# kentsommer/2D-EKF-SLAM

Measured on AMD Instinct MI355X. Metric: EKF steps/sec (propagate+full update) at N landmarks, higher is better.
Workload: dtype f64

## Files before the change

### 2d-ekf-slam_amd/csrc/ekf_api.hip

```cpp
#include <math.h>
#include <stdio.h>
#include <stdlib.h>
#include <string.h>
#include <time.h>

#include <string>
#include <atomic>
#include <mutex>
#include <functional>
#include <vector>
#include <algorithm>

#include "ekf_device.h"
#include "ekf_geometry.h"

#include "ekf_kernels.hip"
#include "ekf_solo.hip"
#include "ekf_rewrite.hip"
#include "ekf_factor.hip"
#include "ekf_pairs.hip"

static thread_local std::string g_last_error;

static int set_error(int code, const char *what) {
// ... 139 lines not shown

extern "C" void ekf_default_params(ekf_params *p) {
    if (!p) return;
    p->sigma_v = 0.01;
    p->sigma_w = 0.04;
    p->gamma_max = 50.0;
    p->gamma_min = 10.0;
    p->cond_limit = 80.0;
    p->max_pending = 16;
    p->log_capacity = 4096;
    p->overlap = -1;
}

static EnvInt env_int(const char *name) {
    EnvInt e;
    if (const char *s = getenv(name)) e.set = true, e.v = atoi(s);
    return e;
}

struct ProcessTunables {
    bool trace;
    bool inline_rec;
};
static const ProcessTunables &process_tunables() {
    static const ProcessTunables t = {env_int("EKF_TRACE").v != 0, env_int("EKF_INLINE_REC").flag(true)};
    return t;
}
static bool trace_on() { return process_tunables().trace; }

static Tunables read_tunables() {
    Tunables t;
    t.overlap = env_int("EKF_OVERLAP");
    t.solo = env_int("EKF_SOLO");
    t.chain_wgs = env_int("EKF_CHAIN_WGS");
    t.solo_long_window = env_int("EKF_SOLO_LONG_WINDOW");
    t.solo_fuse = env_int("EKF_SOLO_FUSE");
    t.chain_one = env_int("EKF_CHAIN_ONE");
    t.chain_helpers = env_int("EKF_CHAIN_HELPERS");
    t.solo_stagger_ticks = env_int("EKF_SOLO_STAGGER_US").set ? env_int("EKF_SOLO_STAGGER_US").v * 100 : 3500;
    t.bm_skew_bytes = getenv("EKF_BM_SKEW") ? atol(getenv("EKF_BM_SKEW")) : 4096;
    t.stream_ring_host = env_int("EKF_STREAM_RING_HOST").flag(false);
    t.balanced_tail = env_int("EKF_BALANCED_TAIL").flag(true);
    t.chain_cus = env_int("EKF_CHAIN_CUS");
    t.inkernel_wait = env_int("EKF_INKERNEL_WAIT").flag(true);
    t.solo_groups = env_int("EKF_SOLO_GROUPS").or_else(1);
    t.flush_alternate = env_int("EKF_FLUSH_ALTERNATE").flag(true);
    t.persist = env_int("EKF_PERSIST").flag(true);
    t.stream = env_int("EKF_STREAM").flag(true);
    t.xcd_map = env_int("EKF_XCD_MAP").flag(true);
    t.batch_interleave = env_int("EKF_BATCH_INTERLEAVE").flag(true);
    t.overlap_serial = getenv("EKF_OVERLAP_SERIAL") != nullptr;
    t.solo_fuse_stagger_ticks = env_int("EKF_SOLO_FUSE_STAGGER_US").v * 100;
    t.inline_rec = process_tunables().inline_rec;
    return t;
}
#define TRACE(msg)                                          \
    do {                                                    \
        if (trace_on()) {                                   \
            fprintf(stderr, "[ekf] %s\n", msg);             \
            fflush(stderr);                                 \
        }                                                   \
    } while (0)

struct PooledStream {
    int device, keep;
    hipStream_t s;
};
static std::mutex g_pool_mu;
static std::vector<PooledStream> g_pool;

static bool pool_take(int device, int keep, hipStream_t *out) {
    std::lock_guard<std::mutex> lk(g_pool_mu);
    for (size_t i = 0; i < g_pool.size(); i++)
        if (g_pool[i].device == device && g_pool[i].keep == keep) {
            *out = g_pool[i].s;
            g_pool.erase(g_pool.begin() + i);
            return true;
        }
    return false;
}

static void pool_drain() {
    std::lock_guard<std::mutex> lk(g_pool_mu);
    for (auto &p : g_pool) {
        if (hipSetDevice(p.device) == hipSuccess) hipStreamDestroy(p.s);
    }
    g_pool.clear();
}

static void pool_give(int device, int keep, hipStream_t s) {
    static bool registered = false;
    std::lock_guard<std::mutex> lk(g_pool_mu);
    if (!registered) {
        atexit(pool_drain);
        registered = true;
    }
    g_pool.push_back({device, keep, s});
}

static int concurrent_kernels_ok(int device, hipStream_t a, hipStream_t b) {
    static std::mutex mu;
    static std::vector<int> cache(64, -1);
    std::lock_guard<std::mutex> lk(mu);
    if (device >= 0 && device < (int)cache.size() && cache[device] >= 0) return cache[device];
    int h[2] = {0, 0}, ok = 0;
    {
// ... 136 lines not shown
    int ndev = 0;
    if (hipGetDeviceCount(&ndev) != hipSuccess || ndev <= 0)
        return set_error(EKF_ERR_NO_DEVICE, "no HIP device: libekfslam_hip has no CPU fallback");
    if (device_id < 0 || device_id >= ndev || device_id >= 64) return set_error(EKF_ERR_BAD_ARG, "bad device_id");
    hipDeviceProp_t prop;
    HIP_TRY(hipGetDeviceProperties(&prop, device_id));
    if (strncmp(prop.gcnArchName, "gfx950", 6) != 0) {
        char buf[256];
        snprintf(buf, sizeof buf, "device %d is %s; this library carries gfx950 code objects only", device_id, prop.gcnArchName);
        return set_error(EKF_ERR_NO_DEVICE, buf);
    }
    HIP_TRY(hipSetDevice(device_id));
    ekf_batch *h = new ekf_batch();
    h->device = device_id;
    int rc = create_impl(h, batch, capacity_landmarks, device_id, params, prop);
    if (rc != EKF_OK) {
        std::string keep = g_last_error;
        ekf_destroy(h);
        (void)hipGetLastError();
        g_last_error = keep;
        return rc;
    }
    *out = h;
    return EKF_OK;
}

static int create_impl(ekf_batch *h, int batch, int capacity_landmarks, int device_id, const ekf_params *params, const hipDeviceProp_t &prop) {
    ekf_default_params(&h->params);
    if (params) h->params = *params;
    h->params_requested = h->params;
    if (h->params.log_capacity < 16) h->params.log_capacity = 16;

    h->tn = read_tunables();
    const Tunables &tn = h->tn;
    const ChainGeometry geo = plan_geometry(batch, capacity_landmarks, h->params, prop.sharedMemPerBlock, tn);
    if (geo.error) return set_error(geo.error, geo.what);
    h->params.max_pending = geo.max_pending;
    h->params.overlap = geo.overlap ? 1 : 0;
    h->overlap = geo.overlap;
    h->solo = geo.solo, h->solo_kernel = geo.solo_kernel, h->solo_long = geo.solo_long, h->solo_fuse = geo.solo_fuse;
    h->chain_wgs = geo.chain_wgs, h->chain_filters = geo.chain_filters, h->chain_threads = geo.chain_threads;
    h->chain_lds = geo.chain_lds, h->chain_one = geo.chain_one;
    EkfDev &dv = h->dv;
    memset(&dv, 0, sizeof dv);
    dv.B = batch;
    dv.Ncap = capacity_landmarks;
    dv.T = geo.T, dv.xs = geo.xs, dv.dn = geo.dn, dv.rows = geo.rows, dv.bm_stride = geo.bm_stride;
    dv.maxp = geo.max_pending, dv.maxpairs = geo.maxpairs, dv.f_stride = geo.f_stride, dv.vs_cap = geo.cache_slots;
    dv.gmax = geo.chain_wgs, dv.lpw = geo.lpw, dv.hpw = geo.hpw, dv.nrec = geo.nrec;
    dv.logcap = h->params.log_capacity;
    dv.gamma_max = h->params.gamma_max;
    dv.gamma_min = h->params.gamma_min;
    dv.spin_limit = 1LL << 24;
    dv.cond_limit = h->params.cond_limit;
    {
        const long double L = h->params.cond_limit;
        long double kappa = L <= 1.0L ? 0.0L : 0.5L - 1.0L / (L * L + 1.0L);
        dv.cond_k2 = (double)(kappa * kappa);
    }

    for (int k = 0; k < 8; k++)
        HIP_TRY(hipFuncSetAttribute((const void *)chain_kernel((k & 4) != 0, (k & 2) != 0, (k & 1) != 0), hipFuncAttributeMaxDynamicSharedMemorySize,
                                    (int)chain_lds_budget(prop.sharedMemPerBlock)));
    {
        const int G = h->chain_wgs;
        int per_cu = 0;
        HIP_TRY(hipOccupancyMaxActiveBlocksPerMultiprocessor(&per_cu, (const void *)chain_kernel(h, false), h->chain_threads, h->chain_lds));
        if (per_cu < 1) return set_error(EKF_ERR_STATE, "the chain kernel does not fit a CU with this capacity / window");
        const int need = h->solo ? 0 : (G * h->chain_filters + per_cu - 1) / per_cu;
        std::lock_guard<std::mutex> lk(g_res_mu);
        if (g_cus_claimed[device_id] + need > prop.multiProcessorCount) {
            char buf[256];
            snprintf(buf, sizeof buf, "this handle's %d chain workgroups need %d CUs, %d of %d are claimed by live handles: they could not all be resident at once",
                     G * h->chain_filters, need, g_cus_claimed[device_id], prop.multiProcessorCount);
            return set_error(EKF_ERR_STATE, buf);
        }
        g_cus_claimed[device_id] += need;
        h->claimed_cus = need;
        h->solo_cus = h->solo ? (h->chain_filters + per_cu - 1) / per_cu : 0;
        if (h->solo_cus > prop.multiProcessorCount) h->solo_cus = prop.multiProcessorCount;
        g_cus_solo[device_id] += h->solo_cus;
        h->ncu = prop.multiProcessorCount;
    }

    if (!pool_take(device_id, -1, &h->s_chain)) {
        TRACE("create: stream");
        HIP_TRY(hipStreamCreateWithFlags(&h->s_chain, hipStreamNonBlocking));
        TRACE("create: stream done");
    }
    const size_t B = batch;
    hipStream_t s = h->s_chain;
    for (const DevArray &a : device_arrays(h)) {
        HIP_TRY(dev_alloc_zero_bytes(a.slot, a.count(batch), a.elem, &h->device_bytes, s));
        if (a.slot != (void **)&dv.Bm[0]) continue;
        if (h->overlap) {
            const size_t skew = (size_t)tn.bm_skew_bytes / sizeof(double);
            HIP_TRY(dev_alloc_zero(&h->bm1_base, B * dv.bm_stride + skew, &h->device_bytes, s));
            dv.Bm[1] = h->bm1_base + skew;
        }
        else dv.Bm[1] = dv.Bm[0];
    }
    TRACE("create: device buffers queued");
    HIP_TRY(hipHostMalloc((void **)&h->mirror_h, B * sizeof(EkfMirror), hipHostMallocMapped));
    memset(h->mirror_h, 0, B * sizeof(EkfMirror));
    HIP_TRY(hipHostGetDevicePointer((void **)&dv.mirror, h->mirror_h, 0));
    HIP_TRY(hipHostMalloc((void **)&h->sctl_h, sizeof(StreamCtl), hipHostMallocMapped));
// ... 1839 lines not shown
```

### 2d-ekf-slam_amd/csrc/ekf_device.h

```cpp
#pragma once
#include <hip/hip_runtime.h>
#include <hip/hip_ext.h>
#include <stdint.h>

#include "../../include/ekfslam_c.h"

#define EKF_INF 999999999999.0
#define EKF_MAX_PENDING 32
#define EKF_MAX_PAIRS (EKF_MAX_PENDING / 2)
#define EKF_CHAIN_MAX_THREADS 256
#define EKF_CHAIN_MAX_WGS 64
#define EKF_CHAIN_MAX_OPS 64
#define EKF_REC_HEAD (16 + 8 * 2 * EKF_MAX_PENDING)
#define EKF_REC_DOUBLES (2 * EKF_REC_HEAD + 16)

enum { OP_NOP = 0, OP_PROP = 1, OP_MEAS = 2, OP_COMPASS = 3, OP_TRUTH = 4, OP_SKIP_SLOT = 5,
       OP_SCRIPT = 6 };
enum { HDR_NONE = 0, HDR_NEW = 1, HDR_OLD = 2, HDR_IGNORE = 3, HDR_COMPASS = 4, HDR_NEW_NOFIT = 5 };

enum { SLOT_DEAD = 0, SLOT_OLD = 1, SLOT_NEW = 2 };
struct SlotMeta {
    int type, ln;
    double S00, S01, S11;
};
// ... 38 lines not shown
#define EKF_STREAM_IDLE_TICKS 10000
enum { EKF_STREAM_RUNNING = 1, EKF_STREAM_EXITING = 2, EKF_STREAM_EXITED = 3 };
enum { EKF_STREAM_END_AFTER = 1, EKF_STREAM_EXIT = 2 };
struct alignas(128) StreamCmd {
    unsigned long long g[18];
};
struct alignas(128) StreamCtl {
    unsigned long long state;
    unsigned long long consumed;
    unsigned long long pad0[14];
    unsigned long long stop;
    unsigned long long pad1[15];
    StreamCmd cmd[EKF_STREAM_RING];
};

struct EkfDev {
    int B, Ncap;
    int xs;
    int dn;
    int T;
    int maxp;
    int maxpairs;
    int vs_cap;
    int logcap;
    int rows;
    int lpw;
    int gmax;
    int hpw;
    int nrec;
    size_t bm_stride;
    size_t f_stride;
    double *x, *R, *D;
    double *Bm[2];
    double *FA, *FB;
    int *n_lm, *n_lm_sweep, *status;
    int *n_lm_flush;
    int *slot_active;
    SlotMeta *slot_meta;
    int *pass_flag;
    unsigned long long *seg_count;
    int *bar;
    long long *dbg;
    double *part;
    StreamCtl *sctl;
    StreamCtl *sring;
    unsigned long long *sfw;
    ekf_decision *log;
    long long *log_count;
    ekf_stats *stats;
    EkfMirror *mirror;
    double gamma_max, gamma_min, cond_limit;
    long long spin_limit;
    double cond_k2;
};

__host__ __device__ inline size_t bm_tile_base(int T, int I, int J) {
    return ((size_t)I * T - ((size_t)I * (I - 1)) / 2 + (size_t)(J - I)) * 4096;
}
__host__ __device__ inline size_t bm_offset(int T, int ip, int jp) {
    int I = ip >> 6, J = jp >> 6;
    size_t t = (size_t)I * T - ((size_t)I * (I - 1)) / 2 + (size_t)(J - I);
    int il = ip & 63, jl = jp & 63;
    int chain = (il >> 4) * 4 + (jl >> 4);
    int rho = il & 15, c = jl & 15;
    int r = rho >> 2, g = rho & 3;
    return t * 4096 + (size_t)chain * 256 + (size_t)(r >> 1) * 128 + (size_t)(g * 16 + c) * 2 + (r & 1);
}

__host__ __device__ inline int lm_tiles(int n) { return (2 * n + 63) >> 6; }

__host__ __device__ inline void bm_tile_coords(int o, int *il, int *jl) {
    const int chain = o >> 8, h = (o >> 7) & 1, lane = (o >> 1) & 63, e = o & 1;
    *il = (chain >> 2) * 16 + (lane >> 4) + 4 * (2 * h + e);
    *jl = (chain & 3) * 16 + (lane & 15);
}

__host__ __device__ inline int remove_row(const int *map, int n_new, int ip) {
    return ip < 2 * n_new ? 2 * map[ip >> 1] + (ip & 1) : -1;
}

enum { RM_ZERO = 0, RM_BM = 1, RM_D = 2 };
struct RmSource {
    int where;
    size_t off;
};
__host__ __device__ inline RmSource remove_source(int T, int dn, int si, int sj) {
    RmSource s;
    if (si < 0 || sj < 0) {
        s.where = RM_ZERO, s.off = 0;
    } else if ((si >> 1) == (sj >> 1)) {
        s.where = RM_D, s.off = (size_t)((si & 1) + (sj & 1)) * dn + (si >> 1);
    } else {
        s.where = RM_BM, s.off = si < sj ? bm_offset(T, si, sj) : bm_offset(T, sj, si);
    }
    return s;
}

struct ReframeItem {
    int off;
    int row[2];
    int col;
    int chain;
};
__host__ __device__ inline ReframeItem reframe_item(int q) {
    ReframeItem it;
    const int chain = q >> 5, h = (q >> 4) & 1, gp = (q >> 3) & 1, c2 = q & 7;
// ... 107 lines not shown
```

### 2d-ekf-slam_amd/csrc/ekf_geometry.h

```cpp
#pragma once
#include <stddef.h>

#include "ekf_device.h"

struct EnvInt {
    bool set = false;
    int v = 0;
    int or_else(int dflt) const { return set ? v : dflt; }
    bool flag(bool dflt) const { return set ? v != 0 : dflt; }
};

struct Tunables {
    EnvInt overlap;
    EnvInt solo;
    EnvInt chain_wgs;
    EnvInt solo_long_window;
    EnvInt solo_fuse;
    EnvInt chain_one;
    EnvInt chain_helpers;
    int solo_stagger_ticks = 3500;
    long bm_skew_bytes = 4096;
    bool stream_ring_host = false;
    bool balanced_tail = true;
    EnvInt chain_cus;
    bool inkernel_wait = true;
    int solo_groups = 1;
    bool flush_alternate = true;
    bool persist = true;
    bool stream = true;
    bool xcd_map = true;
    bool batch_interleave = true;
    bool overlap_serial = false;
    int solo_fuse_stagger_ticks = 0;
    bool inline_rec = true;
};

struct ChainGeometry {
    int error = 0;
    const char *what = nullptr;
    bool overlap = false;
    int max_pending = 0;
    int cache_slots = 0;
    bool solo = false, solo_kernel = false, solo_long = false, solo_fuse = false;
    int chain_wgs = 0;
    int chain_filters = 0;
    int chain_threads = 0;
    size_t chain_lds = 0;
    bool chain_one = false;
    int lpw = 0, hpw = 0, nrec = 0;
    int T = 0, xs = 0, dn = 0, rows = 0, maxpairs = 0;
    size_t bm_stride = 0, f_stride = 0;
};

static inline long chain_lds_budget(size_t lds_per_block) { return (long)lds_per_block - 16384; }

static inline ChainGeometry plan_geometry(int batch, int capacity_landmarks, const ekf_params &params, size_t lds_per_block, const Tunables &tn) {
    ChainGeometry g;
    int maxp = params.max_pending;
    if (maxp < 1) maxp = 1;
    if (maxp > EKF_MAX_PENDING) maxp = EKF_MAX_PENDING;
    g.T = (2 * capacity_landmarks + 63) / 64;
    g.xs = ((3 + 64 * g.T) + 63) / 64 * 64;
    g.dn = 32 * g.T;
    g.bm_stride = (size_t)g.T * (g.T + 1) / 2 * 4096;
    g.rows = 64 * g.T;
    const int max_workers = EKF_CHAIN_MAX_THREADS - 64;
    const long lds_budget = chain_lds_budget(lds_per_block);
    if (lds_budget < 64 * 64) {
        g.error = EKF_ERR_NO_DEVICE, g.what = "device reports too little LDS per workgroup";
        return g;
    }
    int want_overlap = tn.overlap.or_else(params.overlap);
    if (want_overlap < 0) {
        int g_max = batch >= 256 ? 1 : (EKF_CHAIN_MAX_WGS < 256 / batch ? EKF_CHAIN_MAX_WGS : 256 / batch);
        if (g_max < 1) g_max = 1;
        long lpw_min = ((capacity_landmarks + g_max - 1) / g_max + 63) / 64 * 64;
        want_overlap = (lpw_min * maxp * 2 * 32 <= lds_budget) ? 1 : 0;
        size_t T = (2 * (size_t)capacity_landmarks + 63) / 64;
        if ((size_t)batch * (T * (T + 1) / 2) * 4096 * sizeof(double) < ((size_t)8 << 20)) want_overlap = 0;
    }
    g.overlap = want_overlap != 0;
    const int sets_in_lds = g.overlap ? 2 : 1;
    int G = (capacity_landmarks + max_workers - 1) / max_workers;
    int G_lds = (int)((((long)capacity_landmarks + 63) / 64 * 64 * maxp * sets_in_lds * 32 + lds_budget - 1) / lds_budget);
    if (G_lds > G) G = G_lds;
    {
        int G_pref = (capacity_landmarks + 63) / 64;
// ... 61 lines not shown
```

### 2d-ekf-slam_amd/csrc/ekf_kernels.hip

```cpp
#include <stddef.h>
#include "ekf_device.h"
#include "ekf_filter_math.h"

typedef double double4_t __attribute__((ext_vector_type(4)));
typedef double double2_t __attribute__((ext_vector_type(2)));

__device__ __forceinline__ const double *op_record(const double *in, const int *cursor, int k, int B, int b) {
    long op = (cursor ? (long)*cursor : 0L) + k;
    return in + ((size_t)op * B + b) * 8;
}

__device__ __forceinline__ int uni(int v) { return __builtin_amdgcn_readfirstlane(v); }

typedef unsigned int uint4_t __attribute__((ext_vector_type(4)));
__device__ __forceinline__ void st_sc1_b128(void *p, uint4_t v) { asm volatile("global_store_dwordx4 %0, %1, off sc1" : : "v"(p), "v"(v) : "memory"); }

struct RobotState {
    double pose[3];
    double c, s;
    double Prr[9];
    int n_lm, n_sweep;
};

template <int CTRL, int ROW_MASK>
// ... 134 lines not shown
    "s_cmp_gt_u32 %[n], 1\n\ts_cbranch_scc0 Lf1_%=\n\t"                                                                   \
    FOLD_IB(2048, 32)                                                                                                       \
    "s_cmp_gt_u32 %[n], 2\n\ts_cbranch_scc0 LfAB_%=\n"                                                                    \
    "Lfl_%=:\n\t"                                                                                                          \
    FOLD_STEP(FOLD_IC(4096, 64), FOLD_FA, "LfBC_%=")                                                                        \
    FOLD_STEP(FOLD_IA(6144, 96), FOLD_FB, "LfCA_%=")                                                                        \
    FOLD_STEP(FOLD_IB(8192, 128) FOLD_ADV, FOLD_FC, "LfAB_%=")                                                              \
    "s_branch Lfl_%=\n"                                                                                                    \
    "LfBC_%=:\n\t" FOLD_W(4) FOLD_FB FOLD_W(0) FOLD_FC "s_branch Lfe_%=\n"                                                \
    "LfCA_%=:\n\t" FOLD_W(4) FOLD_FC FOLD_W(0) FOLD_FA "s_branch Lfe_%=\n"                                                \
    "LfAB_%=:\n\t" FOLD_W(4) FOLD_FA FOLD_W(0) FOLD_FB "s_branch Lfe_%=\n"                                                \
    "Lf1_%=:\n\t" FOLD_W(0) FOLD_FA                                                                                        \
    "Lfe_%=:\n\t"
#define FOLD_CLOBBERS                                                                                                       \
    "scc", "memory", "v208", "v209", "v210", "v211", "v212", "v213", "v214", "v215", "v216", "v217", "v218", "v219", "v220", "v221", "v222", "v223", \
        "v224", "v225", "v226", "v227", "v228", "v229", "v230", "v231", "v232", "v233", "v234", "v235", "v236", "v237", "v238", "v239", "v240",     \
        "v241", "v242", "v243", "v244", "v245", "v246", "v247", "v248", "v249", "v250", "v251", "v252", "v253", "v254", "v255"

static_assert(sizeof(ChainSeg) == 56 && sizeof(ChainPlan) == 16 + EKF_PLAN_MAX * 56 + 64, "the segment table is read from the kernel-argument segment by offset");
struct ChainKArgs {
    EkfDev dv;
    const double *in;
    const int *cursor;
    ChainPlan plan;
    int b_off;
};
template <bool ONE, bool STREAM = false>
__global__ __launch_bounds__(EKF_CHAIN_MAX_THREADS) void k_chain(EkfDev dv, const double *in, const int *cursor, ChainPlan plan, int b_off) {

    __shared__ ChainLds L;
    __shared__ double recs[EKF_CHAIN_MAX_OPS * 8];
    extern __shared__ __attribute__((aligned(16))) double own_rows[];
    const int g = blockIdx.x, G = gridDim.x;
    const int b = blockIdx.y + b_off;
    const int tid = threadIdx.x;
    const int bd = blockDim.x;
    const bool lead = (g == 0);
    const bool worker = uni(tid >= 64) != 0;
    const bool ctrl = !worker && (tid == 0);
    const int wtid = tid - 64, nw = bd - 64;
    const int xs = dv.xs;
    const int own_lo = g * dv.lpw, own_hi = own_lo + dv.lpw;
    const int lm0 = own_lo + wtid;
    double *x = dv.x + (size_t)b * xs;
    double *R0 = dv.R + (size_t)b * 3 * xs;
    double *Dx = dv.D + (size_t)b * 3 * dv.dn;
    int *bar = dv.bar + (size_t)b * 2;
    double *part = dv.part + (size_t)b * 2 * dv.nrec * EKF_REC_DOUBLES;
    int epoch = 0;
    const int ebase = bar[0];
#ifdef EKF_CHAIN_STAMPS
    unsigned long long stamp_t;
    asm volatile("s_memrealtime %0\n\ts_waitcnt lgkmcnt(0)" : "=s"(stamp_t)::"memory");
    long long stamp_acc[13] = {0, 0, 0, 0, 0, 0, 0, 0, 0, 0, 0, 0, 0};
#endif
    const double *FAb = dv.FA + (size_t)b * 2 * dv.f_stride, *FBb = dv.FB + (size_t)b * 2 * dv.f_stride;
    const int lpw_ = dv.lpw;
    (void)lpw_;
    const int vs_cap = dv.vs_cap;
    auto own_at = [=](int vs, int cmp, int ll) { return (((ll >> 6) * vs_cap + vs) * 2 + (cmp >> 1)) * 128 + (ll & 63) * 2 + (cmp & 1); };
    long long *const dv_dbg = dv.dbg;
    (void)dv_dbg;
    const long long lim_x = xs, lim_R = 3LL * xs, lim_D = 3LL * dv.dn, lim_B = (long long)dv.bm_stride, lim_F = 2LL * (long long)dv.f_stride;
    (void)lim_x, (void)lim_R, (void)lim_D, (void)lim_B, (void)lim_F;
    const int T_ = dv.T, rows_ = dv.rows, dn_ = dv.dn;

    int cur = 0;
    unsigned long long new_mask = 0;
    LmState r0 = {0, 0, {0, 0, 0, 0, 0, 0}, 0, 0, 0};
    const int nseg = plan.nseg;
    typedef __attribute__((address_space(4))) const ChainSeg *SegPtr;
    const SegPtr segs = (SegPtr)((__attribute__((address_space(4))) const char *)__builtin_amdgcn_kernarg_segment_ptr() + offsetof(ChainKArgs, plan) + offsetof(ChainPlan, s));
    const long long last_seq = segs[nseg - 1].seq;
    unsigned long long consumed = STREAM ? (unsigned long long)segs[0].seq : 0ull, n_fw = 0, ack_base = 0;
    const unsigned long long consumed0 = consumed;
    bool end_after = false;
    (void)consumed0, (void)n_fw, (void)ack_base, (void)end_after;
    if (tid == 0) L.abort = 0, L.hflag = -1, L.hflag2 = -1, L.pubflag = 0, L.scmd = 0;
    int fold_no = 0;
    int arrive_base = 0;
    bool arrived = false;
    for (int seg = 0; seg < nseg; seg++) {
    const int k0 = segs[seg].k0, nops = segs[seg].nops, slot0 = segs[seg].slot0, set = segs[seg].set, buf_read = segs[seg].buf_read;
    const int n_prev = segs[seg].n_prev, need_pass = segs[seg].need_pass, drop = segs[seg].drop;
    const double *Bmr = dv.Bm[buf_read] + (size_t)b * dv.bm_stride;
    double *FAc = dv.FA + ((size_t)b * 2 + set) * dv.f_stride;
    double *FBc = dv.FB + ((size_t)b * 2 + set) * dv.f_stride;
    int *act_c = dv.slot_active + ((size_t)b * 2 + set) * dv.maxp;
    const size_t off_c = (size_t)set * dv.f_stride;

    auto lm_load = [=](int lm) {
        LmState st;
        int Li = 3 + 2 * lm;
        st.x0 = x[CK(Li, lim_x)], st.x1 = x[CK(Li + 1, lim_x)];
        for (int i = 0; i < 3; i++) st.rc[i * 2] = R0[CK((size_t)i * xs + Li, lim_R)], st.rc[i * 2 + 1] = R0[CK((size_t)i * xs + Li + 1, lim_R)];
        st.dxx = Dx[CK(lm, lim_D)], st.dxy = Dx[CK(dn_ + lm, lim_D)], st.dyy = Dx[CK(2 * (size_t)dn_ + lm, lim_D)];
        return st;
    };
    auto lm_store = [=](int lm, const LmState &st) {
        int Li = 3 + 2 * lm;
        x[CK(Li, lim_x)] = st.x0, x[CK(Li + 1, lim_x)] = st.x1;
        for (int i = 0; i < 3; i++) R0[CK((size_t)i * xs + Li, lim_R)] = st.rc[i * 2], R0[CK((size_t)i * xs + Li + 1, lim_R)] = st.rc[i * 2 + 1];
        Dx[CK(lm, lim_D)] = st.dxx, Dx[CK(dn_ + lm, lim_D)] = st.dxy, Dx[CK(2 * (size_t)dn_ + lm, lim_D)] = st.dyy;
    };
    auto request_old_inputs = [=](int lm, int lo, double raw[4]) {
        const bool below = lm < lo;
        const int ri = below ? 2 * lm : 2 * lo, ci = below ? 2 * lo : 2 * lm;
        const double *q = Bmr + CK(bm_offset(T_, ri, ci), lim_B - 34);
        raw[0] = q[0], raw[1] = q[2], raw[2] = q[32], raw[3] = q[34];
    };
    auto orient_old_inputs = [=](int lm, int lo, const double raw[4], double p[2][2]) {
        const bool below = lm < lo;
        p[0][0] = raw[0], p[1][1] = raw[3];
        p[0][1] = below ? raw[1] : raw[2], p[1][0] = below ? raw[2] : raw[1];
    };
    auto write_slot = [=](int lm, int slot, double a00, double a01, double a10, double a11, double b00, double b01, double b10, double b11, bool cache_a) {
        const size_t wo = CK(off_c + pair_offset(rows_, 2 * lm, slot >> 1), lim_F - 7) - off_c;
        double *fa = FAc + wo, *fb = FBc + wo;
        double *cr = own_rows + own_at(n_prev + slot, 0, lm - own_lo);
        *(double2_t *)cr = cache_a ? (double2_t){a00, a01} : (double2_t){b00, b01};
        *(double2_t *)(cr + 128) = cache_a ? (double2_t){a10, a11} : (double2_t){b10, b11};
        if ((slot & 1) == 0) {
            *(double4_t *)fa = (double4_t){a00, a01, 0, 0};
            *(double4_t *)(fa + 4) = (double4_t){a10, a11, 0, 0};
            *(double4_t *)fb = (double4_t){b00, b01, 0, 0};
            *(double4_t *)(fb + 4) = (double4_t){b10, b11, 0, 0};
        } else {
            *(double2_t *)(fa + 2) = (double2_t){a00, a01};
            *(double2_t *)(fa + 6) = (double2_t){a10, a11};
            *(double2_t *)(fb + 2) = (double2_t){b00, b01};
            *(double2_t *)(fb + 6) = (double2_t){b10, b11};
        }
// ... 637 lines not shown
                    }
                    wave_argmin(d, i, src);
                    if (lane == 0) L.xd = d, L.xi = i, L.xsrc = src;
                }
                __syncthreads();
                if (L.abort) goto finish;
                gd = L.xd, gi = uni(L.xi), src = uni(L.xsrc);
                epoch++;
                STAMP(2);
            }
            }
            const int w_lo = gi;
            const bool have = (w_lo != 0x7fffffff);
            const double mahal = have ? gd : EKF_INF;
            int hdr;
            if (!have || mahal > dv.gamma_max) hdr = (n_lm_before >= dv.Ncap) ? HDR_NEW_NOFIT : HDR_NEW;
            else if (mahal < dv.gamma_min) hdr = HDR_OLD;
            else hdr = HDR_IGNORE;
            hdr = uni(hdr);
            const int on = (hdr == HDR_NEW || hdr == HDR_OLD) ? 1 : 0;
            const int n_lm_after = n_lm_before + (hdr == HDR_NEW ? 1 : 0);
            if (ctrl) {
                if (lead) {
                    ekf_stats *st = &L.st;
                    if (hdr == HDR_OLD) {
                        st->n_old++;
                        st->nis_sum += mahal;
                        st->nis_count++;
                    } else if (hdr == HDR_IGNORE) {
                        st->n_ignore++;
                    } else {
                        st->n_new++;
                        if (hdr == HDR_NEW_NOFIT) dv.status[b] = EKF_ERR_CAPACITY;
                    }
                    act_c[slot] = on;
                    long long cnt = L.log_count;
                    ekf_decision e;
                    e.decision = hdr == HDR_OLD ? EKF_DECISION_OLD : (hdr == HDR_IGNORE ? EKF_DECISION_IGNORE : EKF_DECISION_NEW);
                    e.matched = have ? 3 + 2 * w_lo : 0;
                    e.mahal = mahal;
                    dv.log[(size_t)b * dv.logcap + (cnt % dv.logcap)] = e;
                    L.dec_buf[L.n_dec++] = e;
                    L.log_count = cnt + 1;
                }
            }

            STAMP(3);
            if (hdr == HDR_OLD) {
                ahead_prop = uni((int)L.ap_tab[op]);
                const int hi = own_hi < n_lm_before ? own_hi : n_lm_before;
                double pf_raw[4] = {0, 0, 0, 0};
                if (worker && lm0 < hi && lm0 != w_lo) request_old_inputs(lm0, w_lo, pf_raw);
                const int nvs = n_prev + slot;
                {
                    const bool slot_thread = tid < nvs;
                    double c4[4] = {0, 0, 0, 0};
                    if (ONE || G > 1) {
                      if (!worker) {
                        const bool cur_thread = slot_thread && tid >= n_prev, w_thread = tid < 16;
                        if (slot_thread && !cur_thread && L.sm[tid].type != SLOT_DEAD) {
                            const size_t off_p = (size_t)(set ^ 1) * dv.f_stride;
                            const double *F = (L.sm[tid].type == SLOT_NEW ? FAb : FBb) + CK(off_p + pair_offset(rows_, 2 * w_lo, tid >> 1), lim_F - 7) + (tid & 1) * 2;
                            c4[0] = F[0], c4[1] = F[1], c4[2] = F[4], c4[3] = F[5];
                        }
                        const unsigned long long *wrec = (const unsigned long long *)(part + ((size_t)((epoch - 1) & 1) * dv.nrec + src) * EKF_REC_DOUBLES);
                        const unsigned long long tag = (unsigned long long)(unsigned)(ebase + epoch) << 32;
                        const unsigned long long *gp = wrec + 2 * (16 + (cur_thread ? tid - n_prev : 0) * 4), *gw = wrec + 2 * (tid & 15);
                        const int ng = cur_thread ? 8 : 0, nwg = w_thread ? 2 : 0;
                        unsigned long long g[10];
                        long spins = 0;
                        for (;;) {
                            unsigned long long bad = 0;
#pragma unroll
                            for (int i = 0; i < 10; i++) {
                                g[i] = tag;
                                if (i < 8 ? i < ng : i - 8 < nwg) g[i] = __hip_atomic_load(i < 8 ? gp + i : gw + (i - 8), __ATOMIC_RELAXED, __HIP_MEMORY_SCOPE_AGENT);
                                bad |= g[i] ^ tag;
                            }
                            if ((bad >> 32) == 0) break;
                            if (++spins > (1L << 22)) {
                                dv.status[b] = EKF_ERR_TIMEOUT, dv.mirror[b].status = EKF_ERR_TIMEOUT;
                                L.abort = 1;
                                break;
                            }
                        }
#ifdef EKF_CHAIN_STAMPS
                        asm volatile("" ::"v"(g[0]), "v"(g[9]));
                        STAMP(12);
#endif
                        if (cur_thread)
                            for (int j = 0; j < 4; j++) c4[j] = __longlong_as_double((long long)((g[2 * j + 1] << 32) | (g[2 * j] & 0xffffffffull)));
                        if (w_thread) L.w[tid] = __longlong_as_double((long long)((g[9] << 32) | (g[8] & 0xffffffffull)));
                      }
                    } else {
                        if constexpr (!ONE) {
                            if (w_lo == best.lm)
                                for (int i = 0; i < 16; i++) L.w[i] = best.w[i];
                            if (slot_thread)
                                for (int j = 0; j < 4; j++) c4[j] = own_rows[own_at(tid, j, w_lo - own_lo)];
                        }
                    }
                    if (slot_thread) {
                        const SlotMeta m = L.sm[tid];
                        double M[4] = {0, 0, 0, 0};
                        if (m.type == SLOT_OLD) {
                            M[0] = -(m.S00 * c4[0] + m.S01 * c4[1]), M[1] = -(m.S00 * c4[2] + m.S01 * c4[3]);
                            M[2] = -(m.S01 * c4[0] + m.S11 * c4[1]), M[3] = -(m.S01 * c4[2] + m.S11 * c4[3]);
                        } else if (m.type == SLOT_NEW && m.ln == w_lo) {
                            M[0] = 1.0, M[3] = 1.0;
                        }
                        for (int j = 0; j < 4; j++) L.loC[tid * 4 + j] = c4[j], L.loM[tid * 4 + j] = M[j];
                    }
                }
                __syncthreads();
                if (L.abort) goto finish;
                STAMP(4);
                const int helpers = uni((bd == 256 && nvs >= 6) ? (lpw_ <= 64 ? 2 : (lpw_ <= 128 ? 1 : 0)) : 0);
                const bool helper_on = helpers != 0;
                const int n_help = helper_on ? nvs / 3 : 0, n_own = nvs - helpers * n_help;
                if (helper_on) fold_no++;
                if (worker) {
                    const OldHdr h = old_header(RS.c, RS.s, L.w);
                    if (helpers == 2 && (wtid >> 6) >= 1) {
                        const int w = wtid >> 6, ll = wtid & 63, first = n_own + (w - 1) * n_help;
                        double q00 = 0, q01 = 0, q10 = 0, q11 = 0;
                        unsigned a0 = lds_off(own_rows + own_at(first, 0, ll)), am = lds_off(L.loM + first * 4);
                        int n = n_help;
                        asm volatile(FOLD_ASM : [p00] "+v"(q00), [p01] "+v"(q01), [p10] "+v"(q10), [p11] "+v"(q11), [a0] "+v"(a0), [am] "+v"(am), [n] "+s"(n) : : FOLD_CLOBBERS);
                        const int at = (w - 1) * 64 + ll;
                        L.hp[at] = q00, L.hp[128 + at] = q01, L.hp[256 + at] = q10, L.hp[384 + at] = q11;
                        __hip_atomic_store(w == 1 ? &L.hflag : &L.hflag2, fold_no, __ATOMIC_RELEASE, __HIP_MEMORY_SCOPE_WORKGROUP);
                    }
                    if (helpers == 1 && (wtid >> 6) == 2) {
                        for (int half = 0; half < 2; half++) {
                            const int ll = half * 64 + (wtid & 63);
                            double q00 = 0, q01 = 0, q10 = 0, q11 = 0;
                            unsigned a0 = lds_off(own_rows + own_at(n_own, 0, ll)), am = lds_off(L.loM + n_own * 4);
                            int n = n_help;
                            asm volatile(FOLD_ASM : [p00] "+v"(q00), [p01] "+v"(q01), [p10] "+v"(q10), [p11] "+v"(q11), [a0] "+v"(a0), [am] "+v"(am), [n] "+s"(n) : : FOLD_CLOBBERS);
                            L.hp[ll] = q00, L.hp[128 + ll] = q01, L.hp[256 + ll] = q10, L.hp[384 + ll] = q11;
                        }
                        __hip_atomic_store(&L.hflag, fold_no, __ATOMIC_RELEASE, __HIP_MEMORY_SCOPE_WORKGROUP);
                    }
                    auto gain_one = [&](int lm, LmState &st, bool prefetched) {
                        double p[2][2] = {{0, 0}, {0, 0}};
                        if (lm == w_lo) {
                            p[0][0] = st.dxx, p[0][1] = st.dxy, p[1][0] = st.dxy, p[1][1] = st.dyy;
                        } else {
                            double raw[4];
                            if (!prefetched) request_old_inputs(lm, w_lo, raw);
                            double pe[2][2] = {{0, 0}, {0, 0}};
                            if (n_own > 0) {
                                unsigned a0 = lds_off(own_rows + own_at(0, 0, lm - own_lo)), am = lds_off(L.loM);
                                int n = n_own;
                                asm volatile(FOLD_ASM
                                             : [p00] "+v"(pe[0][0]), [p01] "+v"(pe[0][1]), [p10] "+v"(pe[1][0]), [p11] "+v"(pe[1][1]), [a0] "+v"(a0), [am] "+v"(am), [n] "+s"(n)
                                             :
                                             : FOLD_CLOBBERS);
                            }
                            for (unsigned long long nm = new_mask; nm; nm &= nm - 1) {
                                const int vs = __builtin_ctzll(nm);
                                if (uni(L.sm[vs].ln) == lm) {
                                    const double *c = L.loC + vs * 4;
                                    pe[0][0] += c[0], pe[0][1] += c[2], pe[1][0] += c[1], pe[1][1] += c[3];
                                }
                            }
#ifdef EKF_CHAIN_STAMPS
                            if (prefetched) {
                                asm volatile("" ::"v"(pe[0][0]), "v"(pe[0][1]), "v"(pe[1][0]), "v"(pe[1][1]));
                                STAMP(9);
                            }
#endif
                            if (prefetched) orient_old_inputs(lm, w_lo, pf_raw, p);
                            else orient_old_inputs(lm, w_lo, raw, p);
#ifdef EKF_CHAIN_STAMPS
                            if (prefetched) {
                                asm volatile("" ::"v"(p[0][0]), "v"(p[0][1]), "v"(p[1][0]), "v"(p[1][1]));
                                STAMP(8);
                            }
#endif
                            for (int a = 0; a < 2; a++)
                                for (int e = 0; e < 2; e++) p[a][e] += pe[a][e];
                            if (helper_on) {
                                while (__hip_atomic_load(&L.hflag, __ATOMIC_ACQUIRE, __HIP_MEMORY_SCOPE_WORKGROUP) != fold_no) {
                                }
                                const int ll = lm - own_lo;
                                p[0][0] += L.hp[ll], p[0][1] += L.hp[128 + ll], p[1][0] += L.hp[256 + ll], p[1][1] += L.hp[384 + ll];
                                if (helpers == 2) {
                                    while (__hip_atomic_load(&L.hflag2, __ATOMIC_ACQUIRE, __HIP_MEMORY_SCOPE_WORKGROUP) != fold_no) {
                                    }
                                    p[0][0] += L.hp[64 + ll], p[0][1] += L.hp[192 + ll], p[1][0] += L.hp[320 + ll], p[1][1] += L.hp[448 + ll];
                                }
                            }
                        }
                        apply_old(lm, st, p, slot, h, RS.Prr, L.w);
                    };
                    if (lm0 < hi) gain_one(lm0, r0, true);
                    if constexpr (!ONE)
                        for (int lm = lm0 + nw; lm < hi; lm += nw) {
                            LmState stm = lm_load(lm);
                            gain_one(lm, stm, false);
                        }
                } else if (tid == 0) {
                    const OldHdr h = old_header(RS.c, RS.s, L.w);
                    double KR[6], TR[6];
                    for (int r = 0; r < 3; r++) old_robot_row(h, RS.Prr + 3 * r, L.w[7 + 2 * r], L.w[8 + 2 * r], KR[r * 2], KR[r * 2 + 1], TR[r * 2], TR[r * 2 + 1]);
// ... 106 lines not shown
                else if (fabs(res2) <= fabs(res3)) res = res2;
                else res = res3;
                double Prr[9];
                for (int i = 0; i < 9; i++) Prr[i] = RS.Prr[i];
                double S = Prr[8] + Rc;
                double invS = 1 / S;
                double KR[3], TR[3];
                for (int r = 0; r < 3; r++) {
                    KR[r] = invS * Prr[r * 3 + 2];
                    TR[r] = S * KR[r];
                }
                for (int r = 0; r < 3; r++) RN.pose[r] = RS.pose[r] + res * KR[r];
                for (int r = 0; r < 3; r++)
                    for (int q = r; q < 3; q++) {
                        double nv = Prr[r * 3 + q] - sym_u(TR[r], 0, KR[r], 0, TR[q], 0, KR[q], 0);
                        RN.Prr[r * 3 + q] = nv;
                        RN.Prr[q * 3 + r] = nv;
                    }
                sincos(RN.pose[2], &RN.s, &RN.c);
                RN.n_lm = RS.n_lm, RN.n_sweep = RS.n_sweep;
                for (int r = 0; r < 3; r++) {
                    L.KR[r * 2] = KR[r], L.KR[r * 2 + 1] = 0;
                    L.TR[r * 2] = TR[r], L.TR[r * 2 + 1] = 0;
                }
                L.S0 = S;
                note_slot(slot, SLOT_OLD, 0, S, 0, 0);
                L.invS = invS;
                L.res0 = res;
                if (lead) act_c[slot] = 1;
            }
            __syncthreads();
            if (worker) {
                const int n_lm = uni(RS.n_lm);
                const int hi = own_hi < n_lm ? own_hi : n_lm;
                if (lm0 < hi) apply_compass(lm0, r0, slot);
                if constexpr (!ONE)
                    for (int lm = lm0 + nw; lm < hi; lm += nw) {
                        LmState stm = lm_load(lm);
                        apply_compass(lm, stm, slot);
                    }
            }
            __syncthreads();
            cur ^= 1;
            slot++;
            continue;
        }
    }
finish:

#ifdef EKF_CHAIN_STAMPS
    if ((tid == 0 || tid == 64) && g == 0 && b == 0)
        for (int i = 0; i < 13; i++)
            if (tid != 0 || i < 8 || i == 12) dv.dbg[(tid == 0 ? 0 : 16) + i] += stamp_acc[i], stamp_acc[i] = 0;
#endif
    if (tid == 0) {
        if (lead) {
            const RobotState &R = L.rs[cur];
            const bool last_seg = seg + 1 == nseg || L.abort;
            if (last_seg && G > 1 && epoch == 0 && !L.abort) {
                long spins = 0;
                while ((int)(__hip_atomic_load(&bar[1], __ATOMIC_RELAXED, __HIP_MEMORY_SCOPE_AGENT) - (arrive_base + G)) < 0) {
                    __builtin_amdgcn_s_sleep(2);
                    if (++spins > (1L << 22)) {
                        dv.status[b] = EKF_ERR_TIMEOUT, dv.mirror[b].status = EKF_ERR_TIMEOUT;
                        break;
                    }
                }
            }
            dv.n_lm_flush[(size_t)b * 2 + set] = R.n_lm;
            if (last_seg) {
                for (int i = 0; i < 3; i++) {
                    x[i] = R.pose[i];
                    for (int j = 0; j < 3; j++) R0[(size_t)i * xs + j] = R.Prr[i * 3 + j];
                }
                dv.n_lm[b] = R.n_lm;
                dv.n_lm_sweep[b] = R.n_sweep;
                dv.stats[b] = L.st;
                dv.log_count[b] = L.log_count;
                publish_mirror((STREAM && plan.stream) ? (long long)consumed : last_seq);
            }
        }
        if (lead && epoch > 0) bar[0] = ebase + epoch;
        if constexpr (STREAM) {
            if (lead && plan.stream) {
                StreamCtl *ctl = dv.sctl;
                __hip_atomic_store(&ctl->consumed, consumed, __ATOMIC_RELAXED, __HIP_MEMORY_SCOPE_SYSTEM);
                __atomic_thread_fence(__ATOMIC_RELEASE);
                __hip_atomic_store(&ctl->state, ((unsigned long long)(unsigned)plan.stream << 2) | EKF_STREAM_EXITED, __ATOMIC_RELAXED, __HIP_MEMORY_SCOPE_SYSTEM);
            }
        }
    }
    if ((seg + 1 == nseg || L.abort) && worker && lm0 < own_hi && lm0 < uni(L.rs[cur].n_lm)) lm_store(lm0, r0);
    if (plan.signal) {
        asm volatile("s_waitcnt vmcnt(0)" ::: "memory");
        __syncthreads();
        if (tid == 0) {
            __builtin_amdgcn_fence(__ATOMIC_RELEASE, "agent");
            __hip_atomic_fetch_add(dv.seg_count + seg, 1ull, __ATOMIC_RELAXED, __HIP_MEMORY_SCOPE_AGENT);
            if (lead && seg + 1 < nseg && !L.abort) {
                EkfMirror *mr = dv.mirror + b;
                for (int i = 0; i < L.n_dec; i++) mr->last[(L.log_count - L.n_dec + i) % EKF_MIRROR_DECISIONS] = L.dec_buf[i];
            }
        }
    } else if (seg + 1 < nseg) {
        __syncthreads();
    }
// ... 345 lines not shown
```

Measured before the change: 39160.

## Fold early previous-slot contributions on helper waves while leader gathers inputs

In the single-chain path with two helper waves, helper waves now load F coefficients, build the M matrices and fold the first n_prev slots (capped by a tunable, default 12) before the workgroup barrier. This overlaps work with the leader wave's gather of current-slot inputs. The remaining slots are then split between the owner and helpers as before, with offsets shifted by the early count. It also moves the old_header computation after the helper dispatch and adds an env knob plus debug stamps. Risks include extra register pressure and changed load balance between waves.

```diff
diff --git a/2d-ekf-slam_amd/csrc/ekf_api.hip b/2d-ekf-slam_amd/csrc/ekf_api.hip
--- a/2d-ekf-slam_amd/csrc/ekf_api.hip
+++ b/2d-ekf-slam_amd/csrc/ekf_api.hip
@@ -215,6 +215,10 @@
     t.overlap_serial = getenv("EKF_OVERLAP_SERIAL") != nullptr;
     t.solo_fuse_stagger_ticks = env_int("EKF_SOLO_FUSE_STAGGER_US").v * 100;
     t.inline_rec = process_tunables().inline_rec;
+    {
+        const int e = env_int("EKF_CHAIN_EARLY_FOLD").or_else(1);
+        t.chain_early_fold = e <= 0 ? 0 : (e == 1 ? EKF_EARLY_FOLD_DEFAULT : e);
+    }
     return t;
 }
 #define TRACE(msg)                                          \
@@ -457,6 +461,7 @@
     dv.gamma_max = h->params.gamma_max;
     dv.gamma_min = h->params.gamma_min;
     dv.spin_limit = 1LL << 24;
+    dv.early_fold = tn.chain_early_fold;
     dv.cond_limit = h->params.cond_limit;
     {
         const long double L = h->params.cond_limit;
diff --git a/2d-ekf-slam_amd/csrc/ekf_device.h b/2d-ekf-slam_amd/csrc/ekf_device.h
--- a/2d-ekf-slam_amd/csrc/ekf_device.h
+++ b/2d-ekf-slam_amd/csrc/ekf_device.h
@@ -114,6 +114,7 @@
     double gamma_max, gamma_min, cond_limit;
     long long spin_limit;
     double cond_k2;
+    int early_fold;
 };
 
 __host__ __device__ inline size_t bm_tile_base(int T, int I, int J) {
diff --git a/2d-ekf-slam_amd/csrc/ekf_geometry.h b/2d-ekf-slam_amd/csrc/ekf_geometry.h
--- a/2d-ekf-slam_amd/csrc/ekf_geometry.h
+++ b/2d-ekf-slam_amd/csrc/ekf_geometry.h
@@ -9,6 +9,8 @@
     int or_else(int dflt) const { return set ? v : dflt; }
     bool flag(bool dflt) const { return set ? v != 0 : dflt; }
 };
+
+#define EKF_EARLY_FOLD_DEFAULT 12
 
 struct Tunables {
     EnvInt overlap;
@@ -33,6 +35,7 @@
     bool overlap_serial = false;
     int solo_fuse_stagger_ticks = 0;
     bool inline_rec = true;
+    int chain_early_fold = EKF_EARLY_FOLD_DEFAULT;
 };
 
 struct ChainGeometry {
diff --git a/2d-ekf-slam_amd/csrc/ekf_kernels.hip b/2d-ekf-slam_amd/csrc/ekf_kernels.hip
--- a/2d-ekf-slam_amd/csrc/ekf_kernels.hip
+++ b/2d-ekf-slam_amd/csrc/ekf_kernels.hip
@@ -210,7 +210,7 @@
 #ifdef EKF_CHAIN_STAMPS
     unsigned long long stamp_t;
     asm volatile("s_memrealtime %0\n\ts_waitcnt lgkmcnt(0)" : "=s"(stamp_t)::"memory");
-    long long stamp_acc[13] = {0, 0, 0, 0, 0, 0, 0, 0, 0, 0, 0, 0, 0};
+    long long stamp_acc[15] = {0, 0, 0, 0, 0, 0, 0, 0, 0, 0, 0, 0, 0, 0, 0};
 #endif
     const double *FAb = dv.FA + (size_t)b * 2 * dv.f_stride, *FBb = dv.FB + (size_t)b * 2 * dv.f_stride;
     const int lpw_ = dv.lpw;
@@ -236,6 +236,7 @@
     (void)consumed0, (void)n_fw, (void)ack_base, (void)end_after;
     if (tid == 0) L.abort = 0, L.hflag = -1, L.hflag2 = -1, L.pubflag = 0, L.scmd = 0;
     int fold_no = 0;
+    const int early_cap_ = dv.early_fold;
     int arrive_base = 0;
     bool arrived = false;
     for (int seg = 0; seg < nseg; seg++) {
@@ -979,13 +980,18 @@
                 double pf_raw[4] = {0, 0, 0, 0};
                 if (worker && lm0 < hi && lm0 != w_lo) request_old_inputs(lm0, w_lo, pf_raw);
                 const int nvs = n_prev + slot;
+                const int helpers = uni((bd == 256 && nvs >= 6) ? (lpw_ <= 64 ? 2 : (lpw_ <= 128 ? 1 : 0)) : 0);
+                int n_early = 0;
+                if constexpr (ONE) n_early = uni((helpers == 2 && n_prev > 0) ? (n_prev < 2 * early_cap_ ? n_prev : 2 * early_cap_) : 0);
+                const int early_a = (n_early + 1) >> 1;
+                double eq00 = 0, eq01 = 0, eq10 = 0, eq11 = 0;
                 {
                     const bool slot_thread = tid < nvs;
                     double c4[4] = {0, 0, 0, 0};
                     if (ONE || G > 1) {
                       if (!worker) {
                         const bool cur_thread = slot_thread && tid >= n_prev, w_thread = tid < 16;
-                        if (slot_thread && !cur_thread && L.sm[tid].type != SLOT_DEAD) {
+                        if (slot_thread && !cur_thread && tid >= n_early && L.sm[tid].type != SLOT_DEAD) {
                             const size_t off_p = (size_t)(set ^ 1) * dv.f_stride;
                             const double *F = (L.sm[tid].type == SLOT_NEW ? FAb : FBb) + CK(off_p + pair_offset(rows_, 2 * w_lo, tid >> 1), lim_F - 7) + (tid & 1) * 2;
                             c4[0] = F[0], c4[1] = F[1], c4[2] = F[4], c4[3] = F[5];
@@ -1018,6 +1024,42 @@
                         if (cur_thread)
                             for (int j = 0; j < 4; j++) c4[j] = __longlong_as_double((long long)((g[2 * j + 1] << 32) | (g[2 * j] & 0xffffffffull)));
                         if (w_thread) L.w[tid] = __longlong_as_double((long long)((g[9] << 32) | (g[8] & 0xffffffffull)));
+                      } else if (n_early > 0 && (wtid >> 6) >= 1) {
+                        const int w = wtid >> 6, ll = wtid & 63;
+                        const int e_first = uni(w == 1 ? 0 : early_a), e_n = uni(w == 1 ? early_a : n_early - early_a);
+                        if (e_n > 0) {
+                            if (ll < e_n) {
+                                const int vs = e_first + ll;
+                                const SlotMeta m = L.sm[vs];
+                                double c4[4] = {0, 0, 0, 0}, M[4] = {0, 0, 0, 0};
+                                if (m.type != SLOT_DEAD) {
+                                    const size_t off_p = (size_t)(set ^ 1) * dv.f_stride;
+                                    const double *F = (m.type == SLOT_NEW ? FAb : FBb) + CK(off_p + pair_offset(rows_, 2 * w_lo, vs >> 1), lim_F - 7) + (vs & 1) * 2;
+                                    c4[0] = F[0], c4[1] = F[1], c4[2] = F[4], c4[3] = F[5];
+                                }
+#ifdef EKF_CHAIN_STAMPS
+                                asm volatile("" ::"v"(c4[0]), "v"(c4[1]), "v"(c4[2]), "v"(c4[3]));
+#endif
+                                if (m.type == SLOT_OLD) {
+                                    M[0] = -(m.S00 * c4[0] + m.S01 * c4[1]), M[1] = -(m.S00 * c4[2] + m.S01 * c4[3]);
+                                    M[2] = -(m.S01 * c4[0] + m.S11 * c4[1]), M[3] = -(m.S01 * c4[2] + m.S11 * c4[3]);
+                                } else if (m.type == SLOT_NEW && m.ln == w_lo) {
+                                    M[0] = 1.0, M[3] = 1.0;
+                                }
+                                for (int j = 0; j < 4; j++) L.loC[vs * 4 + j] = c4[j], L.loM[vs * 4 + j] = M[j];
+                            }
+#ifdef EKF_CHAIN_STAMPS
+                            STAMP(13);
+#endif
+                            asm volatile("s_waitcnt lgkmcnt(0)" ::: "memory");
+                            unsigned a0 = lds_off(own_rows + own_at(e_first, 0, ll)), am = lds_off(L.loM + e_first * 4);
+                            int n = e_n;
+                            asm volatile(FOLD_ASM : [p00] "+v"(eq00), [p01] "+v"(eq01), [p10] "+v"(eq10), [p11] "+v"(eq11), [a0] "+v"(a0), [am] "+v"(am), [n] "+s"(n) : : FOLD_CLOBBERS);
+#ifdef EKF_CHAIN_STAMPS
+                            asm volatile("" ::"v"(eq00), "v"(eq01), "v"(eq10), "v"(eq11));
+                            STAMP(14);
+#endif
+                        }
                       }
                     } else {
                         if constexpr (!ONE) {
@@ -1027,7 +1069,7 @@
                                 for (int j = 0; j < 4; j++) c4[j] = own_rows[own_at(tid, j, w_lo - own_lo)];
                         }
                     }
-                    if (slot_thread) {
+                    if (slot_thread && tid >= n_early) {
                         const SlotMeta m = L.sm[tid];
                         double M[4] = {0, 0, 0, 0};
                         if (m.type == SLOT_OLD) {
@@ -1042,18 +1084,19 @@
                 __syncthreads();
                 if (L.abort) goto finish;
                 STAMP(4);
-                const int helpers = uni((bd == 256 && nvs >= 6) ? (lpw_ <= 64 ? 2 : (lpw_ <= 128 ? 1 : 0)) : 0);
                 const bool helper_on = helpers != 0;
-                const int n_help = helper_on ? nvs / 3 : 0, n_own = nvs - helpers * n_help;
+                const int f_lo = n_early;
+                const int n_help = helper_on ? (nvs - f_lo) / 3 : 0, n_own = nvs - f_lo - helpers * n_help;
                 if (helper_on) fold_no++;
                 if (worker) {
-                    const OldHdr h = old_header(RS.c, RS.s, L.w);
                     if (helpers == 2 && (wtid >> 6) >= 1) {
-                        const int w = wtid >> 6, ll = wtid & 63, first = n_own + (w - 1) * n_help;
-                        double q00 = 0, q01 = 0, q10 = 0, q11 = 0;
-                        unsigned a0 = lds_off(own_rows + own_at(first, 0, ll)), am = lds_off(L.loM + first * 4);
-                        int n = n_help;
-                        asm volatile(FOLD_ASM : [p00] "+v"(q00), [p01] "+v"(q01), [p10] "+v"(q10), [p11] "+v"(q11), [a0] "+v"(a0), [am] "+v"(am), [n] "+s"(n) : : FOLD_CLOBBERS);
+                        const int w = wtid >> 6, ll = wtid & 63, first = f_lo + n_own + (w - 1) * n_help;
+                        double q00 = eq00, q01 = eq01, q10 = eq10, q11 = eq11;
+                        if (n_help > 0) {
+                            unsigned a0 = lds_off(own_rows + own_at(first, 0, ll)), am = lds_off(L.loM + first * 4);
+                            int n = n_help;
+                            asm volatile(FOLD_ASM : [p00] "+v"(q00), [p01] "+v"(q01), [p10] "+v"(q10), [p11] "+v"(q11), [a0] "+v"(a0), [am] "+v"(am), [n] "+s"(n) : : FOLD_CLOBBERS);
+                        }
                         const int at = (w - 1) * 64 + ll;
                         L.hp[at] = q00, L.hp[128 + at] = q01, L.hp[256 + at] = q10, L.hp[384 + at] = q11;
                         __hip_atomic_store(w == 1 ? &L.hflag : &L.hflag2, fold_no, __ATOMIC_RELEASE, __HIP_MEMORY_SCOPE_WORKGROUP);
@@ -1069,6 +1112,7 @@
                         }
                         __hip_atomic_store(&L.hflag, fold_no, __ATOMIC_RELEASE, __HIP_MEMORY_SCOPE_WORKGROUP);
                     }
+                    const OldHdr h = old_header(RS.c, RS.s, L.w);
                     auto gain_one = [&](int lm, LmState &st, bool prefetched) {
                         double p[2][2] = {{0, 0}, {0, 0}};
                         if (lm == w_lo) {
@@ -1078,7 +1122,7 @@
                             if (!prefetched) request_old_inputs(lm, w_lo, raw);
                             double pe[2][2] = {{0, 0}, {0, 0}};
                             if (n_own > 0) {
-                                unsigned a0 = lds_off(own_rows + own_at(0, 0, lm - own_lo)), am = lds_off(L.loM);
+                                unsigned a0 = lds_off(own_rows + own_at(f_lo, 0, lm - own_lo)), am = lds_off(L.loM + f_lo * 4);
                                 int n = n_own;
                                 asm volatile(FOLD_ASM
                                              : [p00] "+v"(pe[0][0]), [p01] "+v"(pe[0][1]), [p10] "+v"(pe[1][0]), [p11] "+v"(pe[1][1]), [a0] "+v"(a0), [am] "+v"(am), [n] "+s"(n)
@@ -1291,6 +1335,10 @@
     if ((tid == 0 || tid == 64) && g == 0 && b == 0)
         for (int i = 0; i < 13; i++)
             if (tid != 0 || i < 8 || i == 12) dv.dbg[(tid == 0 ? 0 : 16) + i] += stamp_acc[i], stamp_acc[i] = 0;
+    if (tid == 128 && g == 0 && b == 0) {
+        dv.dbg[29] += stamp_acc[13], dv.dbg[30] += stamp_acc[14], dv.dbg[31] += stamp_acc[4];
+        stamp_acc[13] = stamp_acc[14] = stamp_acc[4] = 0;
+    }
 #endif
     if (tid == 0) {
         if (lead) {
```

Result: no change. 39310, median of 3 (+0.4%).
